# safijari/yag-slam

Measured on AMD Instinct MI355X. Metric: pose hypotheses/sec, higher is better.
Workload: dtype u8

## Files before the change

include/yagmatch.h:

```cpp
#ifndef YAGMATCH_H
#define YAGMATCH_H

#include <stdint.h>

#ifdef __cplusplus
extern "C" {
#endif

#define YM_VERSION 1

enum {
    YM_OK = 0,
    YM_ERR_INVALID = -1,
    YM_ERR_NO_DEVICE = -2,
    YM_ERR_HIP = -3,
    YM_ERR_UNSUPPORTED = -4,
    YM_ERR_RANGE = -5,
    YM_ERR_BUSY = -6
};

enum { YM_SEM_KARTO = 0, YM_SEM_YAGPY = 1 };

typedef struct ym_config {
    double angle_variance_penalty;
// ... 172 lines not shown
                   double *delta3 , double *precond3 , int32_t *band_used,
                   int32_t *cg_iterations, double *residual, int32_t *flags);
typedef struct ym_opt_params { int32_t iters, exact, max_cg_iters, band ; double lambda0, cg_tol; } ym_opt_params;
typedef struct ym_opt_report { double chi2_initial, chi2_final, lambda_final; int32_t lm_steps, accepted, cg_iterations, band, status; } ym_opt_report;
int ym_graph_optimize(ym_graph *g, const ym_opt_params *p, ym_opt_report *out);

typedef struct ym_grid_info {
    int32_t width, height, pitch;
    int32_t origin_x, origin_y;
    int32_t storage_w, storage_h;
    int32_t roi_x, roi_y, roi_w, roi_h;
    double offset_x, offset_y;
} ym_grid_info;
int ym_debug_grid_info(ym_matcher *m, int item, ym_grid_info *info);
int ym_debug_grid(ym_matcher *m, int item, uint8_t *out, int64_t out_bytes);
int ym_debug_sums(ym_matcher *m, int item, int pass, uint32_t *out, int64_t out_count);
int ym_debug_query_local(ym_matcher *m, int item, double *out_xy, int32_t cap, int32_t *n);
int ym_debug_cells(ym_matcher *m, int item, int32_t *out, int64_t out_count, int32_t *max_n);

int ym_debug_option(ym_matcher *m, int option, int value);

#define YM_DEBUG_COUNTERS 8
int ym_debug_counters(ym_matcher *m, int64_t *out, int32_t count);

int ym_debug_stamps(ym_matcher *m, int enable, uint64_t *out, int32_t count);

int ym_profile_enable(ym_matcher *m, int on);
int ym_profile_read(ym_matcher *m, int which, double *ms_total, int64_t *launches, int reset);
int ym_cache_stats(const ym_matcher *m, int64_t *hits, int64_t *misses);

#ifdef __cplusplus
}
#endif
#endif
```

yag_slam_amd/_capi.py:

```python
import ctypes as C
import os
import subprocess

_HERE = os.path.dirname(os.path.abspath(__file__))
LIB_PATH = os.environ.get("YM_LIB_PATH") or os.path.join(_HERE, "libyagmatch.so")

YM_OK = 0
SEM = {"karto": 0, "yagpy": 1}

EXPORTS = (
    "ym_version", "ym_build_id", "ym_device_count", "ym_last_error", "ym_create", "ym_destroy", "ym_get_config",
    "ym_set_stream", "ym_synchronize", "ym_scan_create", "ym_scans_create", "ym_scans_destroy", "ym_scan_set_pose", "ym_scans_set_poses", "ym_scan_get_pose",
    "ym_scan_size", "ym_scan_structure_trusted", "ym_scan_destroy", "ym_match", "ym_match_scans", "ym_map_sequence", "ym_process_scan", "ym_sequence_stats", "ym_async_slots",
    "ym_match_scans_async", "ym_wait", "ym_match_batch", "ym_batch_create", "ym_batch_destroy", "ym_batch_size",
    "ym_match_pairs", "ym_pairs_create",
    "ym_batch_run_async", "ym_batch_wait", "ym_debug_grid_info",
    "ym_debug_grid", "ym_debug_sums", "ym_debug_query_local", "ym_debug_cells", "ym_debug_option", "ym_debug_stamps",
    "ym_profile_enable",
    "ym_profile_read", "ym_cache_stats", "ym_debug_counters",
    "ym_coarse_dims", "ym_match_slice_begin", "ym_match_slice_finish",
    "ym_occupancy_create", "ym_occupancy_create_counted", "ym_occupancy_get_info", "ym_occupancy_read", "ym_occupancy_read_counts",
    "ym_occupancy_destroy",
    "ym_map_from_occupancy", "ym_map_from_grid", "ym_map_size", "ym_map_read", "ym_map_destroy", "ym_match_map",
    "ym_raymap_create", "ym_raymap_trace", "ym_raymap_trace_each", "ym_raymap_destroy",
    "ym_segments_create", "ym_segments_label_range", "ym_segments_stats", "ym_segments_boundaries", "ym_segments_pairs",
    "ym_segments_destroy", "ym_map_free_space", "ym_segments_from_map", "ym_segments_labels",
    "ym_graph_create", "ym_graph_destroy", "ym_graph_add_nodes", "ym_graph_add_constraints", "ym_graph_size", "ym_graph_set_poses",
    "ym_graph_get_poses", "ym_graph_chi2", "ym_graph_linearise", "ym_graph_solve", "ym_graph_optimize",
)


class YmError(RuntimeError):
    def __init__(self, code, msg):
        super().__init__("libyagmatch error %d: %s" % (code, msg))
        self.code = code


class YmConfig(C.Structure):
    _fields_ = [
        ("angle_variance_penalty", C.c_double),
        ("distance_variance_penalty", C.c_double),
        ("coarse_search_angle_offset", C.c_double),
# ... 139 lines not shown
    L.ym_match_batch.argtypes = [vp, vp, C.POINTER(vp), ip, C.c_int, C.c_int, C.c_int, C.POINTER(YmResult),
                                 C.POINTER(YmResult), ip]
    L.ym_batch_create.restype = vp
    L.ym_batch_create.argtypes = [vp, vp, C.POINTER(vp), ip, C.c_int]
    L.ym_pairs_create.restype = vp
    L.ym_pairs_create.argtypes = [vp, C.POINTER(vp), C.POINTER(vp), ip, C.c_int]
    L.ym_match_pairs.argtypes = [vp, C.POINTER(vp), C.POINTER(vp), ip, C.c_int, C.c_int, C.c_int, C.POINTER(YmResult)]
    L.ym_batch_destroy.argtypes = [vp]
    L.ym_batch_destroy.restype = None
    L.ym_batch_size.argtypes = [vp]
    L.ym_batch_run_async.argtypes = [vp, vp, C.c_int, C.c_int, C.c_int, C.c_int64, vp]
    L.ym_batch_wait.argtypes = [vp, C.c_int, C.POINTER(YmResult), C.POINTER(YmResult), ip]
    L.ym_debug_grid_info.argtypes = [vp, C.c_int, C.POINTER(YmGridInfo)]
    L.ym_debug_grid.argtypes = [vp, C.c_int, C.POINTER(C.c_uint8), C.c_int64]
    L.ym_debug_sums.argtypes = [vp, C.c_int, C.c_int, C.POINTER(C.c_uint32), C.c_int64]
    L.ym_debug_query_local.argtypes = [vp, C.c_int, dp, C.c_int32, ip]
    L.ym_debug_cells.argtypes = [vp, C.c_int, ip, C.c_int64, ip]
    L.ym_debug_option.argtypes = [vp, C.c_int, C.c_int]
    L.ym_debug_stamps.argtypes = [vp, C.c_int, C.POINTER(C.c_uint64), C.c_int32]
    L.ym_profile_enable.argtypes = [vp, C.c_int]
    L.ym_profile_read.argtypes = [vp, C.c_int, dp, C.POINTER(C.c_int64), C.c_int]
    L.ym_cache_stats.argtypes = [vp, C.POINTER(C.c_int64), C.POINTER(C.c_int64)]
    L.ym_debug_counters.argtypes = [vp, C.POINTER(C.c_int64), C.c_int32]
    L.ym_coarse_dims.argtypes = [vp, ip]
    L.ym_scan_structure_trusted.argtypes = [vp, C.c_int]
    L.ym_process_scan.argtypes = [vp, vp, C.POINTER(vp), C.c_int, dp, dp, C.c_int, C.c_int, C.POINTER(YmResult)]
    L.ym_sequence_stats.argtypes = [vp, C.POINTER(C.c_int64), C.POINTER(C.c_int64), C.POINTER(C.c_int64)]
    L.ym_map_sequence.argtypes = [vp, C.POINTER(vp), dp, C.c_int, C.c_int, C.c_int, C.c_int, C.c_int, C.c_int, C.POINTER(YmResult), ip]
    L.ym_match_slice_begin.argtypes = [vp, vp, C.POINTER(vp), C.c_int, C.c_int, C.c_int, C.c_int, C.c_int, vp, vp]
    L.ym_match_slice_finish.argtypes = [vp, C.POINTER(YmResult)]
    L.ym_occupancy_create.restype = vp
    L.ym_occupancy_create.argtypes = [C.POINTER(vp), C.c_int, C.c_double, C.c_double]
    L.ym_occupancy_create_counted.restype = vp
    L.ym_occupancy_create_counted.argtypes = [C.POINTER(vp), C.c_int, C.c_double, C.c_double]
    L.ym_occupancy_get_info.argtypes = [vp, C.POINTER(YmOccupancyInfo)]
    L.ym_occupancy_read.argtypes = [vp, C.POINTER(C.c_uint8), C.c_int64]
    L.ym_occupancy_read_counts.argtypes = [vp, C.POINTER(C.c_uint32), C.POINTER(C.c_uint32), C.c_int64]
    L.ym_occupancy_destroy.argtypes = [vp]
    L.ym_occupancy_destroy.restype = None
    L.ym_map_from_occupancy.restype = vp
    L.ym_map_from_occupancy.argtypes = [vp, C.POINTER(C.c_uint8), C.c_int, C.c_int, C.c_int, C.c_int]
    L.ym_map_from_grid.restype = vp
    L.ym_map_from_grid.argtypes = [vp, dp, C.c_int, C.c_int]
    L.ym_map_size.argtypes = [vp, ip, ip]
    L.ym_map_read.argtypes = [vp, dp, C.c_int64]
    L.ym_map_destroy.argtypes = [vp]
# ... 68 lines not shown
```

yag_slam_amd/csrc/ym_abi_debug.hpp:

```cpp
int ym_debug_grid_info(ym_matcher *m, int item, ym_grid_info *info) {
    if (!m || !info) return set_err(YM_ERR_INVALID, "null argument");
    if (!m->last_valid || item < 0 || item >= m->last_B) return set_err(YM_ERR_INVALID, "no such item in the last call");
    const YmGeom &g = m->last_geom;
    info->width = g.win_w; info->height = g.win_w; info->pitch = g.pitch;
    info->origin_x = g.win_origin; info->origin_y = g.win_origin;
    info->storage_w = g.storage_w; info->storage_h = g.storage_w;
    info->roi_x = g.border; info->roi_y = g.border; info->roi_w = g.roi_w; info->roi_h = g.roi_w;
    YmItemState s;
    DEV_GUARD(m->device);
    HIP_TRY(hipStreamSynchronize(m->stream));
    HIP_TRY(hipMemcpy(&s, m->states.p + item, sizeof s, hipMemcpyDeviceToHost));
    info->offset_x = s.off_x; info->offset_y = s.off_y;
    return YM_OK;
}

int ym_debug_grid(ym_matcher *m, int item, uint8_t *out, int64_t out_bytes) {
    if (!m || !out) return set_err(YM_ERR_INVALID, "null argument");
    if (!m->last_valid || item < 0 || item >= m->last_B) return set_err(YM_ERR_INVALID, "no such item in the last call");
    const int64_t need = (int64_t)m->last_geom.pitch * m->last_geom.win_w;
    if (out_bytes < need) return set_err(YM_ERR_INVALID, "grid buffer too small: need %lld bytes", (long long)need);
    DEV_GUARD(m->device);
    HIP_TRY(hipStreamSynchronize(m->stream));
    HIP_TRY(hipMemcpy(out, m->grid.p + (size_t)item * m->last_grid_stride, (size_t)need, hipMemcpyDeviceToHost));
    return YM_OK;
// ... 154 lines not shown
int ym_sequence_stats(const ym_matcher *m, int64_t *segments, int64_t *faults, int64_t *sync_steps) {
    if (!m || !segments || !faults || !sync_steps) return set_err(YM_ERR_INVALID, "null argument");
    *segments = m->seq_segments; *faults = m->seq_faults; *sync_steps = m->seq_sync_steps;
    return YM_OK;
}

int ym_debug_counters(ym_matcher *m, int64_t *out, int32_t count) {
    if (!m || !out || count < 0) return set_err(YM_ERR_INVALID, "bad argument");
    int64_t v[YM_DEBUG_COUNTERS];
    std::memset(v, 0, sizeof v);
    if (m->yag_counters.p) {
        DEV_GUARD(m->device);
        unsigned long long c[4];
        HIP_TRY(hipStreamSynchronize(m->stream));
        HIP_TRY(hipMemcpy(c, m->yag_counters.p, sizeof c, hipMemcpyDeviceToHost));
        for (int i = 0; i < 4; i++) v[i] = (int64_t)c[i];
    }
    v[4] = m->list_cache_hits;
    v[5] = m->last_corr_form;
    for (int i = 0; i < std::min<int>(count, YM_DEBUG_COUNTERS); i++) out[i] = v[i];
    return YM_OK;
}

int ym_cache_stats(const ym_matcher *m, int64_t *hits, int64_t *misses) {
    if (!m) return set_err(YM_ERR_INVALID, "null matcher");
    if (hits) *hits = m->cache_hits;
    if (misses) *misses = m->cache_misses;
    return YM_OK;
}
```

yag_slam_amd/csrc/ym_host_enqueue.hpp:

```cpp
void enqueue_prepare(ym_matcher *m, const CallPlan &P) {
    ym::PrepareArgs a;
    a.scans = P.d_scans; a.items = P.d_items; a.g = P.g; a.lat = P.lc; a.states = m->states.p; a.qlocal = m->qlocal.p;
    a.cells = m->cells.p; a.bbox = m->bbox.p; a.ctrig = m->ctrig.p; a.hypcell = m->hypcell.p; a.probs = P.probs;
    a.max_n = P.max_n; a.max_base = P.max_base; a.nt_stride = P.nt_stride; a.dim_stride = P.dim_stride; a.stamps = P.stamps;
    a.use_inline = P.inline_desc ? 1 : 0;
    a.pad0 = 0;
    std::memset(&a.inl, 0, sizeof a.inl);
    if (a.use_inline) {
        a.inl.item = P.hi[0];
        for (int i = 0; i < P.nscans; i++) a.inl.scans[i] = P.hs[i];
    }
    a.qnp = m->qnp.p; a.jobs = P.d_jobs; a.job_slot = P.d_job_slot;
    a.fault = nullptr; a.step = 0; a.pad1 = 0;
    for (int k = 0; k < 4; k++) a.cell_box[k] = P.cell_box[k];
    if (P.chain_step) { a.fault = m->seq_fault.p; a.step = P.chain_step; }
    a.tile_max_zero = P.use_tile_list ? m->tile_max.p : nullptr;
    const size_t lds = YM_PREP_LDS_BYTES(P.max_n);
    if (P.split_prepare) {
        if (P.n_jobs > 0) hipLaunchKernelGGL(ym::points_kernel, dim3(P.n_jobs), dim3(YM_POINTS_THREADS), lds, m->stream, a);
        hipLaunchKernelGGL(ym::cells_kernel, dim3(P.max_base + 1, P.B), dim3(256), 0, m->stream, a);
    } else {
        if (P.B == 1 && m->prepare_threads != 512)
            hipLaunchKernelGGL(ym::prepare_kernel<1024>, dim3(P.max_base + 2, P.B), dim3(1024), lds, m->stream, a);
        else
// ... 30 lines not shown
        if (rc) return rc;
        if (m->sel_tables.cap != had) HIP_TRY(hipMemsetAsync(m->sel_tables.p, 0, m->sel_tables.cap * sizeof(unsigned), m->stream));
        if ((rc = m->sel_rec.ensure((size_t)P.B * 12 * 1024))) return rc;
        if ((rc = m->sel_slot.ensure((size_t)P.B * pts))) return rc;
        ym::SelectSplitArgs s;
        s.cells = m->cells.p; s.max_n = P.max_n; s.max_base = P.max_base; s.log2cap = log2cap; s.pad = 0;
        s.keys = m->sel_tables.p; s.mx = s.keys + (size_t)P.B * cap; s.rec = m->sel_rec.p; s.slot_of = m->sel_slot.p; s.stamps = P.stamps;
        const dim3 grid((unsigned)((pts + YM_SELECT_SPLIT_THREADS - 1) / YM_SELECT_SPLIT_THREADS), P.B);
        hipLaunchKernelGGL(ym::select_hash_kernel, grid, dim3(YM_SELECT_SPLIT_THREADS), 0, m->stream, s);
        hipLaunchKernelGGL(ym::select_neighbours_kernel, grid, dim3(YM_SELECT_SPLIT_THREADS), 0, m->stream, s);
        hipLaunchKernelGGL(ym::select_relax_kernel, dim3(P.B), dim3(1024), cap, m->stream, s);
        return YM_OK;
    }
    ym::SelectArgs a;
    a.cells = m->cells.p; a.max_n = P.max_n; a.max_base = P.max_base; a.z2max = m->z2max; a.log2cap = log2cap; a.stamps = P.stamps;
    const size_t lds = (size_t)9 << log2cap;
    hipLaunchKernelGGL(ym::select_kernel<5>, dim3(P.B), dim3(1024), lds, m->stream, a);
    return YM_OK;
}

int enqueue_raster(ym_matcher *m, const CallPlan &P) {
    hipStream_t st = m->stream;
    const YmGeom &g = P.g;
    if (P.use_tile_list) {
        ym::TilesArgs t;
        t.bbox = m->bbox.p; t.tile_list = m->tile_list.p; t.tile_count = m->tile_count.p; t.tile_zero = m->tile_zero.p;
        t.tile_max = m->tile_max.p;
        t.hits = P.use_tile_hits ? m->tile_hits.p : nullptr; t.tile_h = P.tile_h;
        t.hit_limit = m->raster_hits_per_tile > 0 ? std::min(m->raster_hits_per_tile, YM_TILE_HITS) : YM_TILE_HITS;
        t.max_n = P.max_n; t.max_base = P.max_base; t.half_kernel = g.half_kernel;
        t.tiles_x = P.tiles_x; t.tiles_y = P.tiles_y; t.tile_cap = P.tile_cap;
        for (int k = 0; k < 4; k++) t.launch[k] = P.launch[k];
        hipLaunchKernelGGL(ym::tiles_kernel, dim3(P.B), dim3(YM_TILES_THREADS),
                           (size_t)4 * ((P.tiles_x * P.tiles_y + 31) / 32) + (P.use_tile_hits ? (size_t)8 * P.tile_cap : 0), st, t);
    }
    ym::RasterArgs a;
    a.tiles_x = P.tiles_x; a.tiles_y = P.tiles_y; a.tile_x0 = P.launch[0]; a.tile_y0 = P.launch[1]; a.ltx = P.ltx;
    a.tile_list = P.use_tile_list ? m->tile_list.p : nullptr; a.tile_count = m->tile_count.p; a.tile_cap = P.tile_cap;
    a.cells = m->cells.p; a.bbox = m->bbox.p; a.states = m->states.p; a.g = g; a.grid = m->grid.p;
    a.grid_stride = P.grid_stride; a.planes = m->planes.p; a.lut = m->ktab.p; a.max_n = P.max_n; a.max_base = P.max_base; a.stamps = P.stamps;
    a.tile_zero = m->tile_zero.p; a.sub_zero = m->sub_zero.p; a.planes_only = m->raster_planes_only;
    a.n_rowtab = m->raster_no_rowtab ? 0 : m->n_rowtab; a.rowtab = reinterpret_cast<const uint2 *>(m->rowtab.p); a.rowtab_shift = m->rowtab_shift; a.no_planes = P.win_only ? 1 : 0;
    const size_t rlds = YM_RASTER_LDS_BYTES(P.tile_h, g.half_kernel, a.n_rowtab);
    a.tile_max = m->tile_max.p; a.tile_max_host = P.use_tile_list ? m->tile_max_host : nullptr;
    a.hits = (P.use_tile_list && P.use_tile_hits) ? m->tile_hits.p : nullptr; a.lty = P.lty; a.pad0 = 0;
    int rc;
    hipEvent_t ev_k = nullptr;
    if ((rc = prof_begin(m, 1, &ev_k))) return rc;
    if (P.ltx > 0 && P.lty > 0) {
        const int hint = m->tile_max_host ? *reinterpret_cast<volatile int32_t *>(m->tile_max_host) : 0;
        const int gx = m->raster_gx > 0 ? std::min(P.ltx * P.lty, m->raster_gx)
                                        : hint > 0 ? std::min(P.ltx * P.lty, hint + hint / 8 + 2) : P.ltx * P.lty;
        a.first_overflow = gx;
        if (P.use_tile_list) {
            if (P.tile_h == YM_TILE_H_TALL) {
                hipLaunchKernelGGL((ym::raster_kernel<128, false, YM_TILE_H_TALL, true>), dim3(gx, P.B), dim3(128), rlds, st, a);
                if (gx < P.ltx * P.lty) hipLaunchKernelGGL((ym::raster_kernel<128, true, YM_TILE_H_TALL, true>), dim3(4, P.B), dim3(128), rlds, st, a);
            } else {
                hipLaunchKernelGGL((ym::raster_kernel<128, false, YM_TILE_H, true>), dim3(gx, P.B), dim3(128), rlds, st, a);
                if (gx < P.ltx * P.lty) hipLaunchKernelGGL((ym::raster_kernel<128, true, YM_TILE_H, true>), dim3(4, P.B), dim3(128), rlds, st, a);
            }
        } else {
            if (P.tile_h == YM_TILE_H_TALL) hipLaunchKernelGGL((ym::raster_kernel<256, false, YM_TILE_H_TALL, false>), dim3(P.ltx * P.lty, P.B), dim3(256), rlds, st, a);
            else hipLaunchKernelGGL((ym::raster_kernel<256, false, YM_TILE_H, false>), dim3(P.ltx * P.lty, P.B), dim3(256), rlds, st, a);
        }
    }
    return prof_end(m, ev_k);
}
// ... 333 lines not shown
```

yag_slam_amd/csrc/ym_k_common.hpp:

```cpp
#pragma once

namespace ym {

__device__ __forceinline__ double kt_round(double v) { return v >= 0.0 ? floor(v + 0.5) : ceil(v - 0.5); }
__device__ __forceinline__ bool kt_double_equal(double a, double b) {
    double d = a - b;
    return d < 0.0 ? d >= -YM_KT_TOLERANCE : d <= YM_KT_TOLERANCE;
}
__device__ inline double kt_normalize_angle(double angle) {
    while (angle < -YM_KT_PI) {
        if (angle < -YM_KT_2PI) angle += (double)(unsigned int)(angle / -YM_KT_2PI) * YM_KT_2PI;
        else angle += YM_KT_2PI;
    }
    while (angle > YM_KT_PI) {
        if (angle > YM_KT_2PI) angle -= (double)(unsigned int)(angle / YM_KT_2PI) * YM_KT_2PI;
        else angle -= YM_KT_2PI;
    }
    return angle;
}
__device__ inline double kt_normalize_angle_difference(double minuend, double subtrahend) {
    while (minuend - subtrahend < -YM_KT_PI) minuend += YM_KT_2PI;
    while (minuend - subtrahend > YM_KT_PI) minuend -= YM_KT_2PI;
    return minuend;
}
// ... 135 lines not shown
__device__ __forceinline__ int lin_pitch(const YmGeom &g) { return g.kpitch ? g.kpitch : g.pitch; }
__device__ __forceinline__ unsigned cell_value(const YmGeom &g, const uint8_t *grid, unsigned limit, unsigned idx) {
    if (!g.kpitch) return idx < limit ? grid[idx] : 0u;
    if (idx >= (unsigned)(g.kpitch * g.storage_w)) return 0u;
    const unsigned cy = idx / (unsigned)g.kpitch, cx = idx - cy * (unsigned)g.kpitch;
    return cx < (unsigned)g.win_w ? grid[cy * (unsigned)g.pitch + cx] : 0u;
}

__device__ __forceinline__ int hyp_cell(double centre, double start, int i, double step, double off, const YmGeom &g) {
    const double v = start + i * step;
    return world_to_grid(centre + v, off, g.scale) + g.border - g.win_origin;
}

#define YM_BOX_CELLS 16
#define YM_N_BOXES(n) (((n) + YM_BOX_CELLS - 1) / YM_BOX_CELLS)
#define YM_TILE_W 64
#define YM_TILE_H 32
#define YM_TILE_H_TALL 64
#define YM_RASTER_RW ((YM_TILE_W + 2 * YM_MAX_KERNEL_HALF + 63) / 64 + 1)
#define YM_RASTER_GP (YM_TILE_W + 8)
#define YM_RASTER_UNION(th, h, ntab) ((size_t)((th) + 2 * (h)) * YM_RASTER_RW * 8 + (size_t)(ntab) * 1024 > (size_t)(th) * YM_RASTER_GP ? (size_t)((th) + 2 * (h)) * YM_RASTER_RW * 8 + (size_t)(ntab) * 1024 : (size_t)(th) * YM_RASTER_GP)
#define YM_RASTER_LDS_BYTES(th, h, ntab) ((size_t)((th) + 2 * (h)) * YM_RASTER_GP + YM_RASTER_UNION(th, h, ntab) + (size_t)((2 * (h) * (h) + 2 + 15) / 16 * 16))
#define YM_TILE_HITS 64

}
```

yag_slam_amd/csrc/ym_k_prepare.hpp:

```cpp
#pragma once

namespace ym {

#define YM_PREP_LDS_BYTES(max_n) ((size_t)(max_n) * 25 + ((size_t)(max_n) / 64 + 2) * 4 + 16)
#define YM_INLINE_SCANS 16
struct YmInlineDesc {
    YmItem item;
    YmScanRef scans[YM_INLINE_SCANS];
};
struct PrepareArgs {
    const YmScanRef *scans;
    const YmItem *items;
    int32_t use_inline;
    int32_t pad0;
    YmInlineDesc inl;
    YmGeom g;
    YmLattice lat;
    YmItemState *states;
    double2 *qlocal;
    int32_t *qnp;
    int2 *cells;
    int4 *bbox;
    double2 *ctrig;
    int32_t *hypcell;
// ... 552 lines not shown
            if (a.hits) fill[i] = at << 16;
        }
    }
    __syncthreads();
    if (tid == 0) {
        a.tile_count[b] = s_n;
        if (s_n > *reinterpret_cast<volatile int32_t *>(a.tile_max)) atomicMax(a.tile_max, s_n);
    }
    if (!a.hits) return;
    uint16_t *hits = a.hits + (size_t)b * a.tile_cap * YM_TILE_HITS;
    const int n_cchunks = YM_N_BOXES(a.max_n);
    for (int c = tid; c < n_boxes; c += NT) {
        const int4 bb = bbox[c];
        if (bb.x > bb.z) continue;
        const int slot = c / n_cchunks;
        const uint16_t first_cell = (uint16_t)(slot * a.max_n + (c - slot * n_cchunks) * YM_BOX_CELLS);
        const int tx0 = max(lx0, max(bb.x - h, 0) / YM_TILE_W), tx1 = min(lx1, (bb.z + h) / YM_TILE_W);
        const int ty0 = max(ly0, max(bb.y - h, 0) >> th_shift), ty1 = min(ly1, (bb.w + h) >> th_shift);
        for (int ty = ty0; ty <= ty1; ty++)
            for (int tx = tx0; tx <= tx1; tx++) {
                const int i = (ty - ly0) * ltx + (tx - lx0);
                if (cnt[i] > a.hit_limit) continue;
                const int old = atomicAdd(&fill[i], 1);
                hits[(size_t)(old >> 16) * YM_TILE_HITS + (old & 0xffff)] = first_cell;
            }
    }
}

struct SelectArgs {
    int2 *cells;
    int32_t max_n, max_base;
    int32_t z2max;
    int32_t log2cap;
    unsigned long long *stamps;
};

__device__ __forceinline__ unsigned select_key(int x, int y) {
    return ((unsigned)(y + 32768) << 16) | ((unsigned)(x + 32768) & 0xffffu);
}
__device__ __forceinline__ int select_find(const unsigned *keys, unsigned bmask, int shift, unsigned key) {
    unsigned bk = (key * 2654435761u) >> shift;
    for (;;) {
        const uint4 q = *reinterpret_cast<const uint4 *>(keys + 4 * bk);
        if (q.x == key) return (int)(4 * bk);
        if (q.y == key) return (int)(4 * bk + 1);
        if (q.z == key) return (int)(4 * bk + 2);
        if (q.w == key) return (int)(4 * bk + 3);
// ... 374 lines not shown
```

yag_slam_amd/csrc/ym_k_raster.hpp:

```cpp
#pragma once

namespace ym {

struct RasterArgs {
    const int2 *cells;
    const int4 *bbox;
    const YmItemState *states;
    YmGeom g;
    uint8_t *grid;
    size_t grid_stride;
    uint8_t *planes;
    const uint8_t *lut;
    int32_t max_n, max_base;
    uint8_t *tile_zero;
    uint8_t *sub_zero;
    int32_t tiles_x, tiles_y;
    int32_t tile_x0, tile_y0;
    int32_t ltx;
    const uint32_t *tile_list;
    const int32_t *tile_count;
    int32_t tile_cap;
    int32_t first_overflow;
    const uint16_t *hits;
    int32_t lty, pad0;
    const int32_t *tile_max;
    int32_t *tile_max_host;
    int32_t planes_only, n_rowtab;
    int32_t rowtab_shift, no_planes;
    const uint2 *rowtab;
    unsigned long long *stamps;
};

template <int NT, bool OVERFLOW, int TH, bool LISTED>
__global__ __launch_bounds__(NT) void raster_kernel(RasterArgs a) {
    constexpr int TW = YM_TILE_W, HM = YM_MAX_KERNEL_HALF;
    constexpr int MAXHITS = LISTED ? 1 : 256 * TH / 32;
    constexpr int RW = YM_RASTER_RW;
    constexpr int LPR = TW / 8;
    static_assert(RW == (TW + 2 * HM + 63) / 64 + 1, "YM_RASTER_RW");
    constexpr int GP = YM_RASTER_GP;
    extern __shared__ __attribute__((aligned(16))) unsigned char rs_dyn[];
    const int OHh = TH + 2 * a.g.half_kernel;
    unsigned char *grow = rs_dyn;
    unsigned long long *occ = reinterpret_cast<unsigned long long *>(rs_dyn + (size_t)OHh * GP);
    uint2 *rtab = reinterpret_cast<uint2 *>(occ + (size_t)OHh * RW);
    unsigned char *outb = reinterpret_cast<unsigned char *>(occ);
    unsigned char *lut = rs_dyn + YM_RASTER_LDS_BYTES(TH, a.g.half_kernel, a.n_rowtab) - (size_t)((2 * a.g.half_kernel * a.g.half_kernel + 2 + 15) / 16 * 16);
    __shared__ unsigned colany[TW / 8][4];
    __shared__ int s_hits[MAXHITS], s_left[MAXHITS];
    __shared__ int s_nhits;
    const int tid = threadIdx.x;
    const int b = blockIdx.y;
    constexpr int TPT = (5 * 128 + NT - 1) / NT;
    uint2 tq[TPT];
#pragma unroll
    for (int u = 0; u < TPT; u++) tq[u] = (tid + u * NT) < a.n_rowtab * 128 ? a.rowtab[tid + u * NT] : make_uint2(0u, 0u);
    auto one_tile = [&](unsigned entry, int bi, const uint16_t *hl, const unsigned (&hq)[4]) {
    const int tile = (int)(entry & 0x7fffu);
    const int h = a.g.half_kernel;
    const int OW = TW + 2 * h, OH = TH + 2 * h;
    const int tiy = tile / a.tiles_x, tix = tile - tiy * a.tiles_x;
    const int tx0 = tix * TW, ty0 = tiy * TH;
    YM_STAMP(a, 4);
    const int n_cchunks = YM_N_BOXES(a.max_n);
    const int n_boxes = a.max_base * n_cchunks;
    const int4 *bbox = a.bbox + (size_t)bi * n_boxes;
    const int lo_x = tx0 - h, hi_x = tx0 + TW + h - 1, lo_y = ty0 - h, hi_y = ty0 + TH + h - 1;
    uint8_t *grid = a.grid + (size_t)bi * a.grid_stride;
    const int y0 = tid / LPR, x8 = (tid % LPR) * 8;
    const size_t plane_bytes = (size_t)(a.g.pitch / 2) * a.g.win_w;
    uint8_t *planes = a.planes + (size_t)bi * a.grid_stride;
    auto store8 = [&](int y, uint32_t p0, uint32_t p1) {
        if (ty0 + y < a.g.win_w) {
            const uint32_t row = (uint32_t)(ty0 + y), col = (uint32_t)(tx0 + x8);
            if (!a.planes_only) *reinterpret_cast<uint2 *>(grid + (__umul24(row, (uint32_t)a.g.pitch) + col)) = make_uint2(p0, p1);
            if (!a.no_planes) {
                uint8_t *pl = planes + (__umul24(row, (uint32_t)(a.g.pitch / 2)) + col / 2u);
                *reinterpret_cast<uint32_t *>(pl) = __builtin_amdgcn_perm(p1, p0, 0x06040200u);
                *reinterpret_cast<uint32_t *>(pl + plane_bytes) = __builtin_amdgcn_perm(p1, p0, 0x07050301u);
            }
        }
    };
    static_assert(LPR == 8 && (NT / LPR) % 8 == 0, "a wave stores whole bands of eight rows");
    uint8_t *tz = a.tile_zero + ((size_t)bi * a.tiles_y + tiy) * a.tiles_x + tix;
// ... 36 lines not shown
        }
        if (__syncthreads_or(my_hits) == 0) {
            if (tz_old == 0) {
                zero_tile();
                __syncthreads();
                if (tid == 0) *tz = 1;
            }
            return;
        }
        for (int c = tid; c < n_boxes; c += NT) {
            const int4 bb = c == tid ? bb_first : bbox[c];
            if (bb.x <= hi_x && bb.z >= lo_x && bb.y <= hi_y && bb.w >= lo_y) {
                const int at = atomicAdd(&s_nhits, 1);
                if (at < MAXHITS) {
                    const int slot = c / n_cchunks, first = (c - slot * n_cchunks) * YM_BOX_CELLS;
                    s_hits[at] = slot * a.max_n + first;
                    s_left[at] = a.max_n - first;
                }
            }
        }
    }
    const int2 *cells = a.cells + (size_t)bi * a.max_base * a.max_n;
    const int n_cells = a.max_base * a.max_n;
    int2 cc0[4];
    if constexpr (LISTED) {
#pragma unroll
        for (int u = 0; u < 4; u++) {
            const int hi = tid / YM_BOX_CELLS + u * (NT / YM_BOX_CELLS);
            const int ci = (int)hq[u] + (tid % YM_BOX_CELLS);
            cc0[u] = make_int2(YM_CELL_NONE, YM_CELL_NONE);
            if (hi < hn && ci < n_cells) cc0[u] = cells[ci];
        }
    }
    for (int i = tid; i < OH * RW; i += NT) occ[i] = 0ull;
    if (tid < (TW / 8) * 4) (&colany[0][0])[tid] = 0u;
#pragma unroll
    for (int u = 0; u < TPT; u++)
        if ((tid + u * NT) < a.n_rowtab * 128) rtab[tid + u * NT] = tq[u];
    for (int i = tid; i <= 2 * h * h + 1; i += NT) lut[i] = i <= 2 * h * h ? a.lut[i] : (unsigned char)0;
    __syncthreads();
    unsigned *occ32 = reinterpret_cast<unsigned *>(occ);
    int any = 0;
    static_assert(RW == 3, "row_words");
    auto row_words = [](int ly, int word) { int r; asm("v_mad_u32_u24 %0, %1, 6, %2" : "=v"(r) : "v"(ly), "v"(word)); return r; };
    auto stamp = [&](const int2 c2) {
        const int lx = c2.x - lo_x, ly = c2.y - lo_y;
        if (c2.x != YM_CELL_NONE && lx >= 0 && lx < OW && ly >= 0 && ly < OH) {
            atomicOr(&occ32[row_words(ly, lx >> 5)], 1u << (lx & 31));
            any = 1;
        }
    };
    auto walk_boxes = [&]() {
        for (int c0 = 0; c0 < n_boxes; c0 += NT) {
            const int c = c0 + tid;
            bool hit = false;
            if (c < n_boxes) {
                const int4 bb = bbox[c];
                hit = bb.x <= hi_x && bb.z >= lo_x && bb.y <= hi_y && bb.w >= lo_y;
            }
            unsigned long long mask = __ballot(hit);
            while (mask) {
                const int bit = __ffsll((long long)mask) - 1;
                mask &= mask - 1;
                const int chunk = c0 + (tid & ~63) + bit;
                const int slot = chunk / n_cchunks, ci = chunk - slot * n_cchunks;
                const int i = ci * YM_BOX_CELLS + (tid & 63);
                if ((tid & 63) < YM_BOX_CELLS && i < a.max_n) stamp(cells[(size_t)slot * a.max_n + i]);
            }
        }
    };
    int nhits = 0;
    if constexpr (LISTED) {
        nhits = hn;
        if (hn >= 0) {
#pragma unroll
            for (int u = 0; u < 4; u++) stamp(cc0[u]);
            for (int h0 = NT / 4; h0 < hn; h0 += NT / 4) {
                int2 cc[4];
#pragma unroll
                for (int u = 0; u < 4; u++) {
                    const int hi = h0 + tid / YM_BOX_CELLS + u * (NT / YM_BOX_CELLS);
                    cc[u] = make_int2(YM_CELL_NONE, YM_CELL_NONE);
                    if (hi < hn) {
                        const int ci = (int)hl[hi] + (tid % YM_BOX_CELLS);
                        if (ci < n_cells) cc[u] = cells[ci];
                    }
                }
#pragma unroll
                for (int u = 0; u < 4; u++) stamp(cc[u]);
            }
        } else {
            walk_boxes();
        }
    } else {
    nhits = s_nhits;
    if (nhits <= MAXHITS) {
        const int nwork = nhits * YM_BOX_CELLS;
        for (int w0 = 0; w0 < nwork; w0 += 4 * NT) {
            int2 cc[4];
#pragma unroll
            for (int u = 0; u < 4; u++) {
                const int w = w0 + u * NT + tid;
                cc[u] = make_int2(YM_CELL_NONE, YM_CELL_NONE);
                if (w < nwork && (w % YM_BOX_CELLS) < s_left[w / YM_BOX_CELLS]) cc[u] = cells[s_hits[w / YM_BOX_CELLS] + (w % YM_BOX_CELLS)];
            }
#pragma unroll
            for (int u = 0; u < 4; u++) stamp(cc[u]);
        }
    } else {
        walk_boxes();
    }
    }
    any = __syncthreads_or(any);
    YM_STAMP(a, 5);
    if (a.stamps && tid == 0) {
        atomicAdd(a.stamps + 27, 1ull);
        atomicAdd(a.stamps + 28, any ? 1ull : 0ull);
        atomicAdd(a.stamps + 29, (unsigned long long)nhits);
    }
    if (!any) {
        if (tz_old == 0) {
            zero_tile();
            __syncthreads();
            if (tid == 0) *tz = 1;
        }
        return;
    }
    if (tid == 0) *tz = 0;
    if (a.n_rowtab) {
        const unsigned long long gmask = (1ull << (2 * h + 8)) - 1ull;
// ... 63 lines not shown
                    const unsigned long long win = (sw >> q) & wmask;
                    if (win) {
                        const unsigned long long right = win >> h, left = win & lmask;
                        const int dr = right ? (__ffsll((long long)right) - 1) : 255;
                        const int dl = left ? (h - 63 + __clzll((long long)left)) : 255;
                        const unsigned g = (unsigned)(dr < dl ? dr : dl);
                        out[q >> 2] = (out[q >> 2] & ~(0xffu << (8 * (q & 3)))) | (g << (8 * (q & 3)));
                    }
                }
                *reinterpret_cast<uint2 *>(&grow[ry * GP + rx]) = make_uint2(out[0], out[1]);
                atomicOr(&colany[i % LPR][ry >> 5], 1u << (ry & 31));
            }
        }
    }
    __syncthreads();
    YM_STAMP(a, 6);
    typedef unsigned short us2 __attribute__((ext_vector_type(2)));
    const unsigned max_d2 = (unsigned)(2 * h * h);
    const unsigned long long tapmask = (1ull << (2 * h + 1)) - 1ull;
    {
        constexpr int RPW = TH >= 64 ? 64 : TH, GPW = 64 / RPW;
        static_assert(TH % RPW == 0 && TH <= 64 && (TH * LPR) % NT == 0, "a wave takes whole column groups of the tile");
        const int wv = tid >> 6, ln = tid & 63;
        for (int it = 0; it < (TH * LPR) / NT; it++) {
            const int grp = (it * (NT / 64) + wv) * GPW + ln / RPW, y = ln % RPW, gx8 = grp * 8;
            const unsigned *ca = colany[grp];
            const unsigned long long ca_lo = (unsigned long long)ca[0] | (unsigned long long)ca[1] << 32, ca_hi = (unsigned long long)ca[2] | (unsigned long long)ca[3] << 32;
            us2 mn2[4];
#pragma unroll
            for (int q = 0; q < 4; q++) mn2[q] = (us2){0xffff, 0xffff};
            const unsigned long long m64 = 2 * h + 1 <= 32 ? (unsigned long long)(__builtin_amdgcn_alignbit(ca[(y >> 5) + 1], ca[y >> 5], (unsigned)y & 31u) & (unsigned)tapmask)
                                                           : (y ? (ca_lo >> y) | (ca_hi << (64 - y)) : ca_lo) & tapmask;
            uint32_t packed[2] = {0u, 0u};
            if (m64 != 0ull) {
                auto tap = [&](int t) {
                    const int dy = t - h;
                    const uint2 gg = *reinterpret_cast<const uint2 *>(&grow[(y + t) * GP + gx8]);
                    int d2i;
                    asm("v_mul_i32_i24 %0, %1, %1" : "=v"(d2i) : "v"(dy));
                    const unsigned short d2 = (unsigned short)d2i;
                    const us2 dd = (us2){d2, d2};
                    const uint32_t u[4] = {gg.x & 0x00ff00ffu, (gg.x >> 8) & 0x00ff00ffu, gg.y & 0x00ff00ffu, (gg.y >> 8) & 0x00ff00ffu};
#pragma unroll
                    for (int q = 0; q < 4; q++) {
                        us2 gq;
                        __builtin_memcpy(&gq, &u[q], 4);
                        mn2[q] = __builtin_elementwise_min(mn2[q], (us2)(gq * gq + dd));
                    }
                };
                if (2 * h + 1 <= 32) {
                    unsigned m = (unsigned)m64;
                    while (m) {
                        const int t = __ffs((int)m) - 1;
                        m &= m - 1u;
                        tap(t);
                    }
                } else {
                    unsigned long long m = m64;
                    while (m) {
                        const int t = __ffsll((long long)m) - 1;
                        m &= m - 1ull;
                        tap(t);
                    }
                }
                const unsigned short cap = (unsigned short)(max_d2 + 1u);
#pragma unroll
                for (int q = 0; q < 4; q++) mn2[q] = __builtin_elementwise_min(mn2[q], (us2){cap, cap});
                unsigned mn[8];
                mn[0] = mn2[0].x; mn[2] = mn2[0].y; mn[1] = mn2[1].x; mn[3] = mn2[1].y;
                mn[4] = mn2[2].x; mn[6] = mn2[2].y; mn[5] = mn2[3].x; mn[7] = mn2[3].y;
#pragma unroll
                for (int q = 0; q < 8; q++) packed[q >> 2] |= (uint32_t)lut[mn[q]] << (8 * (q & 3));
            }
            *reinterpret_cast<uint2 *>(&outb[y * GP + gx8]) = make_uint2(packed[0], packed[1]);
        }
    }
    __syncthreads();
    for (int y = y0; y < TH; y += NT / LPR) {
        const uint2 v = *reinterpret_cast<const uint2 *>(&outb[y * GP + x8]);
        store_band(y, v.x, v.y, true);
    }
    YM_STAMP(a, 7);
    };
    if constexpr (LISTED) {
        const uint32_t *list = a.tile_list + (size_t)b * a.tile_cap;
        const uint16_t *hits = a.hits ? a.hits + (size_t)b * a.tile_cap * YM_TILE_HITS : nullptr;
        auto load_entry = [&](int e, unsigned &entry, const uint16_t *&hl, unsigned (&hq)[4]) {
            entry = list[e];
            hl = hits ? hits + (size_t)e * YM_TILE_HITS : nullptr;
#pragma unroll
            for (int u = 0; u < 4; u++) hq[u] = hl ? (unsigned)hl[tid / YM_BOX_CELLS + u * (NT / YM_BOX_CELLS)] : 0u;
        };
        static_assert(NT / 4 <= YM_TILE_HITS, "the first round of hit slots must exist");
        if (!OVERFLOW) {
            unsigned entry, hq[4];
            const uint16_t *hl;
            load_entry((int)blockIdx.x, entry, hl, hq);
            const int count = a.tile_count[b];
            if (blockIdx.x == 0 && b == 0 && tid == 0 && a.tile_max_host) *a.tile_max_host = *a.tile_max;
            if ((int)blockIdx.x < count) one_tile(entry, b, hl, hq);
        } else {
            const int count = a.tile_count[b];
            for (int e = a.first_overflow + (int)blockIdx.x; e < count; e += (int)gridDim.x) {
                unsigned entry, hq[4];
                const uint16_t *hl;
                load_entry(e, entry, hl, hq);
                one_tile(entry, b, hl, hq);
                __syncthreads();
            }
        }
    } else {
        const int sy = (int)blockIdx.x / a.ltx, sx = (int)blockIdx.x - sy * a.ltx;
        const unsigned hq[4] = {0u, 0u, 0u, 0u};
        one_tile((unsigned)((a.tile_y0 + sy) * a.tiles_x + a.tile_x0 + (sx + 3 * sy + 5 * b) % a.ltx), b, nullptr, hq);
    }
}

}
```

yag_slam_amd/csrc/ym_kernels.hpp:

```cpp
#pragma once
#include <hip/hip_runtime.h>
#include <math.h>
#include "ym_types.h"

#include "ym_k_common.hpp"
#include "ym_k_prepare.hpp"
#include "ym_k_raster.hpp"
#include "ym_k_correlate.hpp"
#include "ym_k_finish.hpp"
#include "ym_k_region.hpp"
#ifdef YM_EXPERIMENTAL
#include "ym_exp_forms.hpp"
#endif
#include "ym_k_gather.hpp"
#include "ym_k_yagpy.hpp"
#include "ym_k_occupancy.hpp"
#include "ym_k_raytrace.hpp"
#include "ym_k_segments.hpp"
#include "ym_k_segmenter.hpp"
#include "ym_k_posegraph.hpp"
```

Baseline: 13.48 billion.

## Restructure raster hit-slot layout, preload all hit cells, branchless stamping

Hit slots are now written in a thread-major permuted layout so each thread loads its share of a tile's hit list with one vectorized load, and all hit cells are prefetched before the LDS clear instead of looping in rounds. Stamping becomes branchless, using an unsigned range check and a dummy atomic target. The tile-row division is replaced by a host-computed reciprocal multiply, the column pass is specialised at compile time on narrow versus wide kernels, and the LUT copy is done as 32-bit words. This adds register pressure from HR prefetched cells and limits the window to 2048 tile columns.

```diff
diff --git a/include/yagmatch.h b/include/yagmatch.h
--- a/include/yagmatch.h
+++ b/include/yagmatch.h
@@ -218,6 +218,7 @@
 
 #define YM_DEBUG_COUNTERS 8
 int ym_debug_counters(ym_matcher *m, int64_t *out, int32_t count);
+uint32_t ym_debug_tile_recip(int tiles_x);
 
 int ym_debug_stamps(ym_matcher *m, int enable, uint64_t *out, int32_t count);
 
diff --git a/yag_slam_amd/_capi.py b/yag_slam_amd/_capi.py
--- a/yag_slam_amd/_capi.py
+++ b/yag_slam_amd/_capi.py
@@ -17,7 +17,7 @@
     "ym_batch_run_async", "ym_batch_wait", "ym_debug_grid_info",
     "ym_debug_grid", "ym_debug_sums", "ym_debug_query_local", "ym_debug_cells", "ym_debug_option", "ym_debug_stamps",
     "ym_profile_enable",
-    "ym_profile_read", "ym_cache_stats", "ym_debug_counters",
+    "ym_profile_read", "ym_cache_stats", "ym_debug_counters", "ym_debug_tile_recip",
     "ym_coarse_dims", "ym_match_slice_begin", "ym_match_slice_finish",
     "ym_occupancy_create", "ym_occupancy_create_counted", "ym_occupancy_get_info", "ym_occupancy_read", "ym_occupancy_read_counts",
     "ym_occupancy_destroy",
@@ -203,6 +203,8 @@
     L.ym_profile_read.argtypes = [vp, C.c_int, dp, C.POINTER(C.c_int64), C.c_int]
     L.ym_cache_stats.argtypes = [vp, C.POINTER(C.c_int64), C.POINTER(C.c_int64)]
     L.ym_debug_counters.argtypes = [vp, C.POINTER(C.c_int64), C.c_int32]
+    L.ym_debug_tile_recip.argtypes = [C.c_int]
+    L.ym_debug_tile_recip.restype = C.c_uint32
     L.ym_coarse_dims.argtypes = [vp, ip]
     L.ym_scan_structure_trusted.argtypes = [vp, C.c_int]
     L.ym_process_scan.argtypes = [vp, vp, C.POINTER(vp), C.c_int, dp, dp, C.c_int, C.c_int, C.POINTER(YmResult)]
diff --git a/yag_slam_amd/csrc/ym_abi_debug.hpp b/yag_slam_amd/csrc/ym_abi_debug.hpp
--- a/yag_slam_amd/csrc/ym_abi_debug.hpp
+++ b/yag_slam_amd/csrc/ym_abi_debug.hpp
@@ -200,6 +200,8 @@
     return YM_OK;
 }
 
+uint32_t ym_debug_tile_recip(int tiles_x) { return tiles_x >= 1 && tiles_x <= 2048 ? ym::ym_raster_tile_recip(tiles_x) : 0u; }
+
 int ym_cache_stats(const ym_matcher *m, int64_t *hits, int64_t *misses) {
     if (!m) return set_err(YM_ERR_INVALID, "null matcher");
     if (hits) *hits = m->cache_hits;
diff --git a/yag_slam_amd/csrc/ym_host_enqueue.hpp b/yag_slam_amd/csrc/ym_host_enqueue.hpp
--- a/yag_slam_amd/csrc/ym_host_enqueue.hpp
+++ b/yag_slam_amd/csrc/ym_host_enqueue.hpp
@@ -76,6 +76,7 @@
 int enqueue_raster(ym_matcher *m, const CallPlan &P) {
     hipStream_t st = m->stream;
     const YmGeom &g = P.g;
+    if (P.tiles_x > 2048) return set_err(YM_ERR_UNSUPPORTED, "correlation window of %d tile columns: the raster supports 2048", P.tiles_x);
     if (P.use_tile_list) {
         ym::TilesArgs t;
         t.bbox = m->bbox.p; t.tile_list = m->tile_list.p; t.tile_count = m->tile_count.p; t.tile_zero = m->tile_zero.p;
@@ -97,7 +98,7 @@
     a.n_rowtab = m->raster_no_rowtab ? 0 : m->n_rowtab; a.rowtab = reinterpret_cast<const uint2 *>(m->rowtab.p); a.rowtab_shift = m->rowtab_shift; a.no_planes = P.win_only ? 1 : 0;
     const size_t rlds = YM_RASTER_LDS_BYTES(P.tile_h, g.half_kernel, a.n_rowtab);
     a.tile_max = m->tile_max.p; a.tile_max_host = P.use_tile_list ? m->tile_max_host : nullptr;
-    a.hits = (P.use_tile_list && P.use_tile_hits) ? m->tile_hits.p : nullptr; a.lty = P.lty; a.pad0 = 0;
+    a.hits = (P.use_tile_list && P.use_tile_hits) ? m->tile_hits.p : nullptr; a.lty = P.lty; a.tile_recip = ym::ym_raster_tile_recip(P.tiles_x);
     int rc;
     hipEvent_t ev_k = nullptr;
     if ((rc = prof_begin(m, 1, &ev_k))) return rc;
diff --git a/yag_slam_amd/csrc/ym_k_common.hpp b/yag_slam_amd/csrc/ym_k_common.hpp
--- a/yag_slam_amd/csrc/ym_k_common.hpp
+++ b/yag_slam_amd/csrc/ym_k_common.hpp
@@ -181,5 +181,9 @@
 #define YM_RASTER_UNION(th, h, ntab) ((size_t)((th) + 2 * (h)) * YM_RASTER_RW * 8 + (size_t)(ntab) * 1024 > (size_t)(th) * YM_RASTER_GP ? (size_t)((th) + 2 * (h)) * YM_RASTER_RW * 8 + (size_t)(ntab) * 1024 : (size_t)(th) * YM_RASTER_GP)
 #define YM_RASTER_LDS_BYTES(th, h, ntab) ((size_t)((th) + 2 * (h)) * YM_RASTER_GP + YM_RASTER_UNION(th, h, ntab) + (size_t)((2 * (h) * (h) + 2 + 15) / 16 * 16))
 #define YM_TILE_HITS 64
+#define YM_HIT_SPR 8
+#define YM_HIT_POS(s) (((s) % YM_HIT_SPR) * (YM_TILE_HITS / YM_HIT_SPR) + (s) / YM_HIT_SPR)
+__host__ __device__ __forceinline__ uint32_t ym_raster_tile_recip(int tiles_x) { return (uint32_t)(((1u << 26) + (uint32_t)tiles_x - 1u) / (uint32_t)tiles_x); }
+__host__ __device__ __forceinline__ uint32_t ym_tile_row(uint32_t tile, uint32_t recip) { return (uint32_t)(((unsigned long long)tile * recip) >> 26); }
 
 }
diff --git a/yag_slam_amd/csrc/ym_k_prepare.hpp b/yag_slam_amd/csrc/ym_k_prepare.hpp
--- a/yag_slam_amd/csrc/ym_k_prepare.hpp
+++ b/yag_slam_amd/csrc/ym_k_prepare.hpp
@@ -598,7 +598,7 @@
                 const int i = (ty - ly0) * ltx + (tx - lx0);
                 if (cnt[i] > a.hit_limit) continue;
                 const int old = atomicAdd(&fill[i], 1);
-                hits[(size_t)(old >> 16) * YM_TILE_HITS + (old & 0xffff)] = first_cell;
+                hits[(size_t)(old >> 16) * YM_TILE_HITS + YM_HIT_POS(old & 0xffff)] = first_cell;
             }
     }
 }
diff --git a/yag_slam_amd/csrc/ym_k_raster.hpp b/yag_slam_amd/csrc/ym_k_raster.hpp
--- a/yag_slam_amd/csrc/ym_k_raster.hpp
+++ b/yag_slam_amd/csrc/ym_k_raster.hpp
@@ -22,13 +22,20 @@
     int32_t tile_cap;
     int32_t first_overflow;
     const uint16_t *hits;
-    int32_t lty, pad0;
+    int32_t lty;
+    uint32_t tile_recip;
     const int32_t *tile_max;
     int32_t *tile_max_host;
     int32_t planes_only, n_rowtab;
     int32_t rowtab_shift, no_planes;
     const uint2 *rowtab;
     unsigned long long *stamps;
+};
+
+template <int N>
+struct HitSlots {
+    uint32_t w[(N + 1) / 2];
+    __device__ __forceinline__ unsigned get(int u) const { return (u & 1) ? w[u >> 1] >> 16 : w[u >> 1] & 0xffffu; }
 };
 
 template <int NT, bool OVERFLOW, int TH, bool LISTED>
@@ -52,14 +59,20 @@
     const int tid = threadIdx.x;
     const int b = blockIdx.y;
     constexpr int TPT = (5 * 128 + NT - 1) / NT;
+    const int n_tab_entries = a.n_rowtab * 128;
     uint2 tq[TPT];
 #pragma unroll
-    for (int u = 0; u < TPT; u++) tq[u] = (tid + u * NT) < a.n_rowtab * 128 ? a.rowtab[tid + u * NT] : make_uint2(0u, 0u);
-    auto one_tile = [&](unsigned entry, int bi, const uint16_t *hl, const unsigned (&hq)[4]) {
+    for (int u = 0; u < TPT; u++) {
+        tq[u] = make_uint2(0u, 0u);
+        if ((u + 1) * NT <= n_tab_entries) tq[u] = a.rowtab[tid + u * NT];
+        else if (u * NT < n_tab_entries && tid + u * NT < n_tab_entries) tq[u] = a.rowtab[tid + u * NT];
+    }
+    constexpr int HR = LISTED ? YM_TILE_HITS / (NT / YM_BOX_CELLS) : 1;
+    auto one_tile = [&](unsigned entry, int bi, const HitSlots<HR> &hq) {
     const int tile = (int)(entry & 0x7fffu);
     const int h = a.g.half_kernel;
     const int OW = TW + 2 * h, OH = TH + 2 * h;
-    const int tiy = tile / a.tiles_x, tix = tile - tiy * a.tiles_x;
+    const int tiy = (int)ym_tile_row((uint32_t)tile, a.tile_recip), tix = tile - tiy * a.tiles_x;
     const int tx0 = tix * TW, ty0 = tiy * TH;
     YM_STAMP(a, 4);
     const int n_cchunks = YM_N_BOXES(a.max_n);
@@ -142,33 +155,42 @@
     }
     const int2 *cells = a.cells + (size_t)bi * a.max_base * a.max_n;
     const int n_cells = a.max_base * a.max_n;
-    int2 cc0[4];
+    constexpr int SPR = NT / YM_BOX_CELLS;
+    int2 cc0[HR];
+    unsigned dead0 = 0u;
     if constexpr (LISTED) {
 #pragma unroll
-        for (int u = 0; u < 4; u++) {
-            const int hi = tid / YM_BOX_CELLS + u * (NT / YM_BOX_CELLS);
-            const int ci = (int)hq[u] + (tid % YM_BOX_CELLS);
-            cc0[u] = make_int2(YM_CELL_NONE, YM_CELL_NONE);
-            if (hi < hn && ci < n_cells) cc0[u] = cells[ci];
+        for (int u = 0; u < HR; u++) {
+            if (u * SPR < hn) {
+                const int hi = u * SPR + tid / YM_BOX_CELLS;
+                const int ci = (int)hq.get(u) + (tid % YM_BOX_CELLS);
+                dead0 |= (hi < hn && ci < n_cells) ? 0u : 128u << u;
+                cc0[u] = *reinterpret_cast<const int2 *>(reinterpret_cast<const char *>(cells) + (uint32_t)min(ci, n_cells - 1) * 8u);
+            }
         }
     }
     for (int i = tid; i < OH * RW; i += NT) occ[i] = 0ull;
     if (tid < (TW / 8) * 4) (&colany[0][0])[tid] = 0u;
 #pragma unroll
-    for (int u = 0; u < TPT; u++)
-        if ((tid + u * NT) < a.n_rowtab * 128) rtab[tid + u * NT] = tq[u];
-    for (int i = tid; i <= 2 * h * h + 1; i += NT) lut[i] = i <= 2 * h * h ? a.lut[i] : (unsigned char)0;
+    for (int u = 0; u < TPT; u++) {
+        if ((u + 1) * NT <= n_tab_entries) rtab[tid + u * NT] = tq[u];
+        else if (u * NT < n_tab_entries && tid + u * NT < n_tab_entries) rtab[tid + u * NT] = tq[u];
+    }
+#pragma unroll 1
+    for (int i = tid; i < (2 * h * h + 2 + 3) / 4; i += NT) reinterpret_cast<uint32_t *>(lut)[i] = reinterpret_cast<const uint32_t *>(a.lut)[i];
     __syncthreads();
     unsigned *occ32 = reinterpret_cast<unsigned *>(occ);
     int any = 0;
     static_assert(RW == 3, "row_words");
     auto row_words = [](int ly, int word) { int r; asm("v_mad_u32_u24 %0, %1, 6, %2" : "=v"(r) : "v"(ly), "v"(word)); return r; };
-    auto stamp = [&](const int2 c2) {
-        const int lx = c2.x - lo_x, ly = c2.y - lo_y;
-        if (c2.x != YM_CELL_NONE && lx >= 0 && lx < OW && ly >= 0 && ly < OH) {
-            atomicOr(&occ32[row_words(ly, lx >> 5)], 1u << (lx & 31));
-            any = 1;
-        }
+    static_assert(YM_CELL_NONE == INT32_MIN && TH * RW * 2 >= 64 && TW + 2 * HM < 128, "stamp");
+    auto stamp = [&](const int2 c2, unsigned dead) {
+        const unsigned lx = (unsigned)(c2.x - lo_x) | dead, ly = (unsigned)(c2.y - lo_y);
+        const int word = row_words((int)ly, (int)(lx >> 5));
+        const bool in = lx < (unsigned)OW && ly < (unsigned)OH;
+        const unsigned bit = in ? 1u << (lx & 31u) : 0u;
+        atomicOr(&occ32[in ? word : (tid & 63)], bit);
+        any |= (int)bit;
     };
     auto walk_boxes = [&]() {
         for (int c0 = 0; c0 < n_boxes; c0 += NT) {
@@ -185,7 +207,7 @@
                 const int chunk = c0 + (tid & ~63) + bit;
                 const int slot = chunk / n_cchunks, ci = chunk - slot * n_cchunks;
                 const int i = ci * YM_BOX_CELLS + (tid & 63);
-                if ((tid & 63) < YM_BOX_CELLS && i < a.max_n) stamp(cells[(size_t)slot * a.max_n + i]);
+                if ((tid & 63) < YM_BOX_CELLS && i < a.max_n) stamp(cells[(size_t)slot * a.max_n + i], 0u);
             }
         }
     };
@@ -194,21 +216,8 @@
         nhits = hn;
         if (hn >= 0) {
 #pragma unroll
-            for (int u = 0; u < 4; u++) stamp(cc0[u]);
-            for (int h0 = NT / 4; h0 < hn; h0 += NT / 4) {
-                int2 cc[4];
-#pragma unroll
-                for (int u = 0; u < 4; u++) {
-                    const int hi = h0 + tid / YM_BOX_CELLS + u * (NT / YM_BOX_CELLS);
-                    cc[u] = make_int2(YM_CELL_NONE, YM_CELL_NONE);
-                    if (hi < hn) {
-                        const int ci = (int)hl[hi] + (tid % YM_BOX_CELLS);
-                        if (ci < n_cells) cc[u] = cells[ci];
-                    }
-                }
-#pragma unroll
-                for (int u = 0; u < 4; u++) stamp(cc[u]);
-            }
+            for (int u = 0; u < HR; u++)
+                if (u * SPR < hn) stamp(cc0[u], dead0 & (128u << u));
         } else {
             walk_boxes();
         }
@@ -225,7 +234,7 @@
                 if (w < nwork && (w % YM_BOX_CELLS) < s_left[w / YM_BOX_CELLS]) cc[u] = cells[s_hits[w / YM_BOX_CELLS] + (w % YM_BOX_CELLS)];
             }
 #pragma unroll
-            for (int u = 0; u < 4; u++) stamp(cc[u]);
+            for (int u = 0; u < 4; u++) stamp(cc[u], 0u);
         }
     } else {
         walk_boxes();
@@ -335,15 +344,21 @@
         constexpr int RPW = TH >= 64 ? 64 : TH, GPW = 64 / RPW;
         static_assert(TH % RPW == 0 && TH <= 64 && (TH * LPR) % NT == 0, "a wave takes whole column groups of the tile");
         const int wv = tid >> 6, ln = tid & 63;
+        auto column_pass = [&](auto narrow) {
+        constexpr bool NARROW = decltype(narrow)::value;
         for (int it = 0; it < (TH * LPR) / NT; it++) {
             const int grp = (it * (NT / 64) + wv) * GPW + ln / RPW, y = ln % RPW, gx8 = grp * 8;
             const unsigned *ca = colany[grp];
-            const unsigned long long ca_lo = (unsigned long long)ca[0] | (unsigned long long)ca[1] << 32, ca_hi = (unsigned long long)ca[2] | (unsigned long long)ca[3] << 32;
             us2 mn2[4];
 #pragma unroll
             for (int q = 0; q < 4; q++) mn2[q] = (us2){0xffff, 0xffff};
-            const unsigned long long m64 = 2 * h + 1 <= 32 ? (unsigned long long)(__builtin_amdgcn_alignbit(ca[(y >> 5) + 1], ca[y >> 5], (unsigned)y & 31u) & (unsigned)tapmask)
-                                                           : (y ? (ca_lo >> y) | (ca_hi << (64 - y)) : ca_lo) & tapmask;
+            unsigned long long m64;
+            if constexpr (NARROW) {
+                m64 = (unsigned long long)(__builtin_amdgcn_alignbit(ca[(y >> 5) + 1], ca[y >> 5], (unsigned)y & 31u) & (unsigned)tapmask);
+            } else {
+                const unsigned long long ca_lo = (unsigned long long)ca[0] | (unsigned long long)ca[1] << 32, ca_hi = (unsigned long long)ca[2] | (unsigned long long)ca[3] << 32;
+                m64 = (y ? (ca_lo >> y) | (ca_hi << (64 - y)) : ca_lo) & tapmask;
+            }
             uint32_t packed[2] = {0u, 0u};
             if (m64 != 0ull) {
                 auto tap = [&](int t) {
@@ -361,7 +376,7 @@
                         mn2[q] = __builtin_elementwise_min(mn2[q], (us2)(gq * gq + dd));
                     }
                 };
-                if (2 * h + 1 <= 32) {
+                if constexpr (NARROW) {
                     unsigned m = (unsigned)m64;
                     while (m) {
                         const int t = __ffs((int)m) - 1;
@@ -387,6 +402,9 @@
             }
             *reinterpret_cast<uint2 *>(&outb[y * GP + gx8]) = make_uint2(packed[0], packed[1]);
         }
+        };
+        if (2 * h + 1 <= 32) column_pass(std::true_type{});
+        else column_pass(std::false_type{});
     }
     __syncthreads();
     for (int y = y0; y < TH; y += NT / LPR) {
@@ -398,34 +416,41 @@
     if constexpr (LISTED) {
         const uint32_t *list = a.tile_list + (size_t)b * a.tile_cap;
         const uint16_t *hits = a.hits ? a.hits + (size_t)b * a.tile_cap * YM_TILE_HITS : nullptr;
-        auto load_entry = [&](int e, unsigned &entry, const uint16_t *&hl, unsigned (&hq)[4]) {
+        static_assert(NT / YM_BOX_CELLS == YM_HIT_SPR && HR * YM_HIT_SPR == YM_TILE_HITS && (HR * 2) % 8 == 0, "YM_HIT_POS is this kernel's thread-to-slot map");
+        auto load_entry = [&](int e, unsigned &entry, HitSlots<HR> &hq) {
             entry = list[e];
-            hl = hits ? hits + (size_t)e * YM_TILE_HITS : nullptr;
-#pragma unroll
-            for (int u = 0; u < 4; u++) hq[u] = hl ? (unsigned)hl[tid / YM_BOX_CELLS + u * (NT / YM_BOX_CELLS)] : 0u;
+            if (hits) {
+                const uint2 *src = reinterpret_cast<const uint2 *>(hits + ((uint32_t)e * YM_TILE_HITS + (uint32_t)(tid / YM_BOX_CELLS) * HR));
+                if constexpr (HR == 8) {
+                    const uint4 v = *reinterpret_cast<const uint4 *>(src);
+                    hq.w[0] = v.x; hq.w[1] = v.y; hq.w[2] = v.z; hq.w[3] = v.w;
+                } else {
+#pragma unroll
+                    for (int u = 0; u < HR / 4; u++) { const uint2 v = src[u]; hq.w[2 * u] = v.x; hq.w[2 * u + 1] = v.y; }
+                }
+            }
         };
-        static_assert(NT / 4 <= YM_TILE_HITS, "the first round of hit slots must exist");
         if (!OVERFLOW) {
-            unsigned entry, hq[4];
-            const uint16_t *hl;
-            load_entry((int)blockIdx.x, entry, hl, hq);
+            unsigned entry;
+            HitSlots<HR> hq;
+            load_entry((int)blockIdx.x, entry, hq);
             const int count = a.tile_count[b];
             if (blockIdx.x == 0 && b == 0 && tid == 0 && a.tile_max_host) *a.tile_max_host = *a.tile_max;
-            if ((int)blockIdx.x < count) one_tile(entry, b, hl, hq);
+            if ((int)blockIdx.x < count) one_tile(entry, b, hq);
         } else {
             const int count = a.tile_count[b];
             for (int e = a.first_overflow + (int)blockIdx.x; e < count; e += (int)gridDim.x) {
-                unsigned entry, hq[4];
-                const uint16_t *hl;
-                load_entry(e, entry, hl, hq);
-                one_tile(entry, b, hl, hq);
+                unsigned entry;
+                HitSlots<HR> hq;
+                load_entry(e, entry, hq);
+                one_tile(entry, b, hq);
                 __syncthreads();
             }
         }
     } else {
         const int sy = (int)blockIdx.x / a.ltx, sx = (int)blockIdx.x - sy * a.ltx;
-        const unsigned hq[4] = {0u, 0u, 0u, 0u};
-        one_tile((unsigned)((a.tile_y0 + sy) * a.tiles_x + a.tile_x0 + (sx + 3 * sy + 5 * b) % a.ltx), b, nullptr, hq);
+        const HitSlots<HR> hq{};
+        one_tile((unsigned)((a.tile_y0 + sy) * a.tiles_x + a.tile_x0 + (sx + 3 * sy + 5 * b) % a.ltx), b, hq);
     }
 }
 
diff --git a/yag_slam_amd/csrc/ym_kernels.hpp b/yag_slam_amd/csrc/ym_kernels.hpp
--- a/yag_slam_amd/csrc/ym_kernels.hpp
+++ b/yag_slam_amd/csrc/ym_kernels.hpp
@@ -1,6 +1,7 @@
 #pragma once
 #include <hip/hip_runtime.h>
 #include <math.h>
+#include <type_traits>
 #include "ym_types.h"
 
 #include "ym_k_common.hpp"
```

Result: faster. 13.72 billion (median of 6 runs) (+1.8%).
